# SciML/NonlinearSolve.jl

Hardware: AMD Instinct MI355X
Metric: newton_steps_per_sec (higher is better)
Workload: dtype f64; 1 GPU; bratu2d_1024x1024_newtonraphson_gmres30_fixedwork_csr_spmv; unknowns_global=1048576, unknowns_per_gpu=1048576, arnoldi_steps_per_newton_step=30, ortho=sstep_auto_auto, parallelism=row-range x1, comm=none

## Files before the change

nonlinearsolve.jl_amd/csrc/nk_powers.hip:

```cpp
#include <algorithm>
#include <stdlib.h>
#include <vector>

#include "nk_internal.h"

constexpr int PW_T = 1024;
constexpr int PW_HALO = 1024;
constexpr int PW_FLAG_STRIDE = 16;
constexpr int PW_NXCD = 8;

struct pw_args {
  int nrows, nb, s, stall;
  const int32_t *rowptr, *col;
  const double *val;
  const double *x0;
  double *Y;
  int64_t ldy;
  const double *scal_first, *scal_rest, *theta;
  const int *d_skip;
  uint64_t *flags;
  uint64_t base;
  uint64_t *err;
  int ns;
  double c_lap;
  const double *diag;
  int seg_len, ring;
  struct {
    int up, dn;
    const int32_t *halo_vl;
    double *push_up, *push_dn;
    uint64_t *flag_up, *flag_dn;
    const double *recv_up, *recv_dn;
    const uint64_t *myflag_up, *myflag_dn;
    uint64_t *err;
    int ebuf;
  } pr;
};

constexpr int PW_NST = 12, PW_STP = 16;
__device__ unsigned long long *g_pw_stamp = nullptr;
#ifdef NK_PW_STAMPS
#define PW_STAMP(p, i) do { if (t == 0 && (p) < PW_STP) s_pw_st[(p) * PW_NST + (i)] = wall_clock64(); } while (0)
#else
#define PW_STAMP(p, i) do { } while (0)
#endif

__device__ __forceinline__ int pw_band_of(int bid, int nb) {
  const int q = nb / PW_NXCD, r = nb % PW_NXCD;
  const int x = bid % PW_NXCD, k = bid / PW_NXCD;
  return x * q + (x < r ? x : r) + k;
}
__device__ __forceinline__ void pw_store_sc1(double *p, double v) {
  __hip_atomic_store(reinterpret_cast<unsigned long long *>(p), (unsigned long long)__double_as_longlong(v), __ATOMIC_RELAXED,
                     __HIP_MEMORY_SCOPE_AGENT);
}
__device__ __forceinline__ double pw_load_sc1(const double *p) {
  return __longlong_as_double((long long)__hip_atomic_load(reinterpret_cast<const unsigned long long *>(p), __ATOMIC_RELAXED,
                                                           __HIP_MEMORY_SCOPE_AGENT));
}
__device__ __forceinline__ bool pw_wait(const uint64_t *f, uint64_t target, uint64_t *err) {
  if (__hip_atomic_load(f, __ATOMIC_RELAXED, __HIP_MEMORY_SCOPE_AGENT) >= target) return true;
  const unsigned long long t0 = wall_clock64(), lim = err[1];
  for (unsigned it = 1;; ++it) {
    __builtin_amdgcn_s_sleep(1);
    if (__hip_atomic_load(f, __ATOMIC_RELAXED, __HIP_MEMORY_SCOPE_AGENT) >= target) return true;
    if ((it & 63u) == 0) {
      if (__hip_atomic_load(err, __ATOMIC_RELAXED, __HIP_MEMORY_SCOPE_SYSTEM) != 0) return false;
      if (wall_clock64() - t0 > lim) {
        __hip_atomic_store(err, (uint64_t)1, __ATOMIC_RELAXED, __HIP_MEMORY_SCOPE_SYSTEM);
        return false;
      }
    }
  }
}
__device__ __forceinline__ bool pw_wait_peer(const uint64_t *f, uint64_t target, uint64_t *perr, uint64_t *err) {
  if (__hip_atomic_load(f, __ATOMIC_ACQUIRE, __HIP_MEMORY_SCOPE_SYSTEM) >= target) return true;
  const unsigned long long t0 = wall_clock64(), lim = nk_peer_timeout(perr);
  for (unsigned it = 1;; ++it) {
    __builtin_amdgcn_s_sleep(1);
    if (__hip_atomic_load(f, __ATOMIC_ACQUIRE, __HIP_MEMORY_SCOPE_SYSTEM) >= target) return true;
    if ((it & 63u) == 0) {
      if (__hip_atomic_load(err, __ATOMIC_RELAXED, __HIP_MEMORY_SCOPE_SYSTEM) != 0) return false;
      if (__hip_atomic_load(perr, __ATOMIC_RELAXED, __HIP_MEMORY_SCOPE_AGENT) > 4 || wall_clock64() - t0 > lim) {
        atomicAdd((unsigned long long *)perr, 1ull);
        __hip_atomic_store(err, (uint64_t)1, __ATOMIC_RELAXED, __HIP_MEMORY_SCOPE_SYSTEM);
        return false;
      }
    }
  }
}
__device__ __forceinline__ void pw_store_sys(double *p, double v) {
  __hip_atomic_store(reinterpret_cast<unsigned long long *>(p), (unsigned long long)__double_as_longlong(v), __ATOMIC_RELAXED,
                     __HIP_MEMORY_SCOPE_SYSTEM);
}
__device__ __forceinline__ double pw_load_sys(const double *p) {
  return __longlong_as_double((long long)__hip_atomic_load(reinterpret_cast<const unsigned long long *>(p), __ATOMIC_RELAXED,
                                                           __HIP_MEMORY_SCOPE_SYSTEM));
}
__device__ __forceinline__ double pw_uniform(double x) {
  const unsigned long long u = (unsigned long long)__double_as_longlong(x);
  const unsigned lo = __builtin_amdgcn_readfirstlane((unsigned)u), hi = __builtin_amdgcn_readfirstlane((unsigned)(u >> 32));
  return __longlong_as_double((long long)(((unsigned long long)hi << 32) | lo));
}
template <int RPT>
__device__ __forceinline__ constexpr int pw_slice(int q) {
  return q == 0 ? 0 : (q == 1 ? RPT - 1 : q - 1);
}

template <int RPT, int W, int GEN, bool PEER = false>
__global__ __launch_bounds__(PW_T) void k_spmv_powers(const pw_args a) {
  if (a.d_skip != nullptr && *a.d_skip != 0) return;
  extern __shared__ double pw_x[];
  __shared__ int s_abort;
#ifdef NK_PW_STAMPS
  __shared__ unsigned long long s_pw_st[PW_STP * PW_NST];
  for (int i = threadIdx.x; i < PW_STP * PW_NST; i += PW_T) s_pw_st[i] = 0;
#endif
  constexpr int RB = PW_T * RPT, XN = RB + 2 * PW_HALO;
  constexpr int NBND = RPT > 1 ? 2 : 1;
  const int t = threadIdx.x;
  const int b = pw_band_of(blockIdx.x, a.nb);
  const int r0 = b * RB;
  double *xa = pw_x, *xb = pw_x + XN;
  const bool pup = PEER && b == 0 && a.pr.up != 0, pdn = PEER && b == a.nb - 1 && a.pr.dn != 0;

  double v[RPT][W];
  int ci[RPT][W];
  int len[RPT];
  if constexpr (GEN == 1) {
    static_assert(W >= 5, "the 5-point stencil needs five slots per row");
#pragma unroll
    for (int i = 0; i < RPT; ++i) {
      const int r = r0 + t + PW_T * i;
      const int rc = r < a.nrows ? r : a.nrows - 1;
      const int gj = rc / a.ns, gi = rc - gj * a.ns;
      const double dd = a.diag[rc];
      const int base = rc - (r0 - PW_HALO), own = PW_HALO + t + PW_T * i;
      const bool hs = gj > 0, hw = gi > 0, he = gi + 1 < a.ns, hn = gj + 1 < a.ns;
      const int pW = hs ? 1 : 0, pC = pW + (hw ? 1 : 0), pE = pC + 1, pN = pE + (he ? 1 : 0), n = pN + (hn ? 1 : 0);
      const double off = -a.c_lap, ctr = 4.0 * a.c_lap - dd;
#pragma unroll
      for (int j = 0; j < W; ++j) {
        double vv = 0.0;
        int cc = own;
        if (hs && j == 0) { vv = off; cc = base - a.ns; }
        if (hw && j == pW) { vv = off; cc = base - 1; }
        if (j == pC) { vv = ctr; cc = base; }
        if (he && j == pE) { vv = off; cc = base + 1; }
        if (hn && j == pN) { vv = off; cc = base + a.ns; }
        v[i][j] = vv;
        ci[i][j] = cc;
      }
      len[i] = r < a.nrows ? n : 0;
    }
  } else if constexpr (W > 8) {
#pragma unroll
    for (int i = 0; i < RPT; ++i) {
      const int r = r0 + t + PW_T * i;
      const int rc = r < a.nrows ? r : a.nrows - 1;
      const int k0 = a.rowptr[rc], k1 = a.rowptr[rc + 1];
      len[i] = r < a.nrows ? k1 - k0 : 0;
#pragma unroll
      for (int j = 0; j < W; ++j) {
        v[i][j] = a.val[k0 + j];
        int c = a.col[k0 + j];
        if (PEER && (pup || pdn) && j < len[i] && c >= a.nrows) c = a.pr.halo_vl[c - a.nrows];
        ci[i][j] = (j < len[i]) ? c - (r0 - PW_HALO) : PW_HALO + t + PW_T * i;
      }
    }
  } else {
    double *sv = pw_x;
    int *sc = reinterpret_cast<int *>(pw_x + (size_t)PW_T * W);
#pragma unroll
    for (int i = 0; i < RPT; ++i) {
      const int rfirst = r0 + PW_T * i;
      const int r = rfirst + t;
      const int rc = r < a.nrows ? r : a.nrows - 1;
      const int k0 = a.rowptr[rc], k1 = a.rowptr[rc + 1];
      const int rl = rfirst < a.nrows ? (rfirst + PW_T <= a.nrows ? rfirst + PW_T : a.nrows) : rfirst;
      const int kb = rfirst < a.nrows ? a.rowptr[rfirst] : 0, ke = rfirst < a.nrows ? a.rowptr[rl] : 0;
      len[i] = r < a.nrows ? k1 - k0 : 0;
#pragma unroll
      for (int j = 0; j < W; ++j) {
        const int e = t + PW_T * j;
        if (kb + e < ke) { sv[e] = a.val[kb + e]; sc[e] = a.col[kb + e]; }
      }
      __syncthreads();
#pragma unroll
      for (int j = 0; j < W; ++j) {
        const int e = (j < len[i]) ? k0 - kb + j : 0;
        const double vv = sv[e];
        int c = sc[e];
        if (PEER && (pup || pdn) && j < len[i] && c >= a.nrows) c = a.pr.halo_vl[c - a.nrows];
        v[i][j] = (j < len[i]) ? vv : 0.0;
        ci[i][j] = (j < len[i]) ? c - (r0 - PW_HALO) : PW_HALO + t + PW_T * i;
      }
      __syncthreads();
    }
  }
  for (int idx = t; idx < XN; idx += PW_T) {
    const int g = r0 - PW_HALO + idx;
    xa[idx] = (g >= 0 && g < a.nrows) ? a.x0[g] : 0.0;
    xb[idx] = 0.0;
  }
  if (t == 0) s_abort = 0;
  __syncthreads();
  if (PEER && (pup || pdn)) {
    if (pup) pw_store_sys(a.pr.push_up + (size_t)a.pr.ebuf * PW_T + t, a.x0[t]);
    if (pdn) pw_store_sys(a.pr.push_dn + (size_t)a.pr.ebuf * PW_T + t, a.x0[a.nrows - PW_T + t]);
    __threadfence_system();
    __syncthreads();
    if (t == 0 && pup) __hip_atomic_store(a.pr.flag_up, a.base, __ATOMIC_RELEASE, __HIP_MEMORY_SCOPE_SYSTEM);
    if (t == 64 && pdn) __hip_atomic_store(a.pr.flag_dn, a.base, __ATOMIC_RELEASE, __HIP_MEMORY_SCOPE_SYSTEM);
    if (t == 0 && pup && !pw_wait_peer(a.pr.myflag_up, a.base, a.pr.err, a.err)) s_abort = 1;
    if (t == 64 && pdn && !pw_wait_peer(a.pr.myflag_dn, a.base, a.pr.err, a.err)) s_abort = 1;
    __syncthreads();
    if (s_abort) return;
    if (pup) xa[t] = pw_load_sys(a.pr.recv_up + (size_t)a.pr.ebuf * PW_T + t);
    if (pdn) xa[PW_HALO + RB + t] = pw_load_sys(a.pr.recv_dn + (size_t)a.pr.ebuf * PW_T + t);
    __syncthreads();
  }

  const bool shifted = a.theta != nullptr;
  const double os_first = pw_uniform(a.scal_first ? *a.scal_first : 1.0), os_rest = pw_uniform(a.scal_rest ? *a.scal_rest : 1.0);
  double th = pw_uniform(shifted ? a.theta[0] : 0.0);
  for (int p = 0; p < a.s; ++p) {
    const double *xin = (p & 1) ? xb : xa;
    double *xout = (p & 1) ? xa : xb;
    const double *osp = (p == 0) ? a.scal_first : a.scal_rest;
    const double os = (p == 0) ? os_first : os_rest;
    double *ycol = a.Y + (int64_t)p * a.ldy;
    const bool pub = p + 1 < a.s;
    const size_t boff = (size_t)(a.pr.ebuf + ((p + 1) & 1)) * PW_T + t;
    PW_STAMP(p, 0);
#pragma unroll
    for (int q = 0; q < RPT; ++q) {
      const int i = pw_slice<RPT>(q);
      const int lr = t + PW_T * i, r = r0 + lr;
      constexpr bool BATCH = RPT * W < 30;
      double xv[BATCH ? W : 1], xo = 0.0;
      if constexpr (BATCH) {
#pragma unroll
        for (int j = 0; j < W; ++j) xv[j] = xin[ci[i][j]];
        xo = xin[PW_HALO + lr];
        __builtin_amdgcn_sched_barrier(0);
      }
      double sum = 0.0;
#pragma unroll
      for (int j = 0; j < W; ++j) {
        double xj;
        if constexpr (BATCH) xj = xv[j]; else xj = xin[ci[i][j]];
        const double pr = v[i][j] * xj;
        sum = (j < len[i]) ? sum + pr : sum;
      }
      if constexpr (!BATCH) xo = xin[PW_HALO + lr];
      double out = shifted ? sum - th * xo : sum;
      out = osp ? os * out : out;
      if (r < a.nrows) {
        xout[PW_HALO + lr] = out;
        if (q < NBND) pw_store_sc1(ycol + r, out);
        else ycol[r] = out;
      }
      if (PEER && pub) {
        if (pup && i == 0) pw_store_sys(a.pr.push_up + boff, out);
        if (pdn && i == RPT - 1) pw_store_sys(a.pr.push_dn + boff, out);
      }
      if (q == NBND - 1) PW_STAMP(p, 1);
      if (pub && q == NBND - 1) {
        if (PEER && (pup || pdn)) __threadfence_system();
        asm volatile("s_waitcnt vmcnt(0)" ::: "memory");
        PW_STAMP(p, 2);
        __syncthreads();
        PW_STAMP(p, 3);
        if (t == 0 && !(a.stall && b == 0))
          __hip_atomic_store(a.flags + (size_t)b * PW_FLAG_STRIDE, a.base + (uint64_t)p + 1, __ATOMIC_RELAXED,
                             __HIP_MEMORY_SCOPE_AGENT);
        if (PEER) {
          if (t == 64 && pup) __hip_atomic_store(a.pr.flag_up, a.base + (uint64_t)p + 1, __ATOMIC_RELEASE, __HIP_MEMORY_SCOPE_SYSTEM);
          if (t == 128 && pdn) __hip_atomic_store(a.pr.flag_dn, a.base + (uint64_t)p + 1, __ATOMIC_RELEASE, __HIP_MEMORY_SCOPE_SYSTEM);
        }
      }
    }
    PW_STAMP(p, 4);
    if (!pub) break;
    if (t == 0) {
      if (b > 0) {
        if (!pw_wait(a.flags + (size_t)(b - 1) * PW_FLAG_STRIDE, a.base + (uint64_t)p + 1, a.err)) s_abort = 1;
      } else if (PEER && pup) {
        if (!pw_wait_peer(a.pr.myflag_up, a.base + (uint64_t)p + 1, a.pr.err, a.err)) s_abort = 1;
      }
    }
    PW_STAMP(p, 5);
    if (t == 64) {
      if (b + 1 < a.nb) {
        if (!pw_wait(a.flags + (size_t)(b + 1) * PW_FLAG_STRIDE, a.base + (uint64_t)p + 1, a.err)) s_abort = 1;
      } else if (PEER && pdn) {
        if (!pw_wait_peer(a.pr.myflag_dn, a.base + (uint64_t)p + 1, a.pr.err, a.err)) s_abort = 1;
      }
    }
    __syncthreads();
    PW_STAMP(p, 6);
    if (s_abort) return;
    {
      const int gu = r0 - PW_HALO + t, gd = r0 + RB + t;
      double hu = 0.0, hd = 0.0;
      if (b > 0) hu = pw_load_sc1(ycol + gu);
      else if (PEER && pup) hu = pw_load_sys(a.pr.recv_up + boff);
      if (gd < a.nrows) hd = pw_load_sc1(ycol + gd);
      else if (PEER && pdn) hd = pw_load_sys(a.pr.recv_dn + boff);
      th = pw_uniform(shifted ? a.theta[p + 1] : 0.0);
#ifdef NK_PW_STAMPS
      asm volatile("s_waitcnt vmcnt(0)" ::: "memory");
      PW_STAMP(p, 7);
#endif
      xout[t] = hu;
      xout[PW_HALO + RB + t] = hd;
    }
    __syncthreads();
    PW_STAMP(p, 9);
  }
#ifdef NK_PW_STAMPS
  __syncthreads();
  if (g_pw_stamp != nullptr)
    for (int i = t; i < PW_STP * PW_NST; i += PW_T) g_pw_stamp[(size_t)b * PW_STP * PW_NST + i] = s_pw_st[i];
#endif
}

template <int RPS, int W, int SEG>
__global__ __launch_bounds__(PW_T) void k_spmv_powers_seg(const pw_args a) {
  if (a.d_skip != nullptr && *a.d_skip != 0) return;
  extern __shared__ double pw_x[];
  __shared__ int s_abort;
  constexpr int RB = PW_T * RPS, XS = RB + 2 * PW_HALO, XN = SEG * XS, NSL = SEG * RPS;
  static_assert(W <= 8, "the slices are staged through LDS");
  const int t = threadIdx.x;
  const int b = pw_band_of(blockIdx.x, a.nb);
  const int M = a.seg_len, b0 = b * RB;
  const bool ring = a.ring != 0;
  double *xa = pw_x, *xb = pw_x + XN;

  double v[NSL][W];
  int ci[NSL][W];
  int len[NSL];
  {
    double *sv = pw_x;
    int *sc = reinterpret_cast<int *>(pw_x + (size_t)PW_T * W);
#pragma unroll
    for (int i = 0; i < NSL; ++i) {
      const int sg = i / RPS, j = i % RPS;
      const int lfirst = b0 + PW_T * j;
      const bool any = lfirst < M;
      const bool valid = lfirst + t < M;
      const int rfirst = sg * M + lfirst, r = rfirst + t;
      const int rc = valid ? r : (any ? sg * M + M - 1 : 0);
      const int k0 = a.rowptr[rc], k1 = a.rowptr[rc + 1];
      const int rl = any ? sg * M + (lfirst + PW_T <= M ? lfirst + PW_T : M) : 0;
      const int kb = any ? a.rowptr[rfirst] : 0, ke = any ? a.rowptr[rl] : 0;
      len[i] = valid ? k1 - k0 : 0;
#pragma unroll
      for (int jj = 0; jj < W; ++jj) {
        const int e = t + PW_T * jj;
        if (kb + e < ke) { sv[e] = a.val[kb + e]; sc[e] = a.col[kb + e]; }
      }
      __syncthreads();
#pragma unroll
      for (int jj = 0; jj < W; ++jj) {
        const int e = (jj < len[i]) ? k0 - kb + jj : 0;
        const double vv = sv[e];
        const int c = sc[e];
        const int sgc = SEG > 1 ? c / M : 0;
        int d = c - sgc * M - b0;
        if (ring) d = d < -PW_HALO ? d + M : (d >= RB + PW_HALO ? d - M : d);
        v[i][jj] = (jj < len[i]) ? vv : 0.0;
        ci[i][jj] = (jj < len[i]) ? sgc * XS + PW_HALO + d : sg * XS + PW_HALO + PW_T * j + t;
      }
      __syncthreads();
    }
  }
  for (int idx = t; idx < XN; idx += PW_T) {
    const int sg = idx / XS;
    int l = b0 - PW_HALO + (idx - sg * XS);
    if (ring) l = l < 0 ? l + M : (l >= M ? l - M : l);
    xa[idx] = (l >= 0 && l < M) ? a.x0[sg * M + l] : 0.0;
    xb[idx] = 0.0;
  }
  if (t == 0) s_abort = 0;
  __syncthreads();

  const bool shifted = a.theta != nullptr;
  const int nup = b > 0 ? b - 1 : (ring ? a.nb - 1 : -1), ndn = b + 1 < a.nb ? b + 1 : (ring ? 0 : -1);
  for (int p = 0; p < a.s; ++p) {
    const double *xin = (p & 1) ? xb : xa;
    double *xout = (p & 1) ? xa : xb;
    const double *osp = (p == 0) ? a.scal_first : a.scal_rest;
    const double os = osp ? *osp : 1.0;
    const double th = shifted ? a.theta[p] : 0.0;
    double *ycol = a.Y + (int64_t)p * a.ldy;
    const bool pub = p + 1 < a.s;
#pragma unroll
    for (int i = 0; i < NSL; ++i) {
      const int sg = i / RPS, j = i % RPS;
      const int lrow = b0 + PW_T * j + t, own = sg * XS + PW_HALO + PW_T * j + t;
      double sum = 0.0;
#pragma unroll
      for (int jj = 0; jj < W; ++jj) {
        const double pr = v[i][jj] * xin[ci[i][jj]];
        sum = (jj < len[i]) ? sum + pr : sum;
      }
      double out = shifted ? sum - th * xin[own] : sum;
      out = osp ? os * out : out;
      if (lrow < M) {
        xout[own] = out;
        if (pub && (j == 0 || j == RPS - 1)) pw_store_sc1(ycol + sg * M + lrow, out);
        else ycol[sg * M + lrow] = out;
      }
    }
    if (!pub) break;
    asm volatile("s_waitcnt vmcnt(0)" ::: "memory");
    __syncthreads();
    if (t == 0 && !(a.stall && b == 0))
      __hip_atomic_store(a.flags + (size_t)b * PW_FLAG_STRIDE, a.base + (uint64_t)p + 1, __ATOMIC_RELAXED, __HIP_MEMORY_SCOPE_AGENT);
    if (t == 0 && nup >= 0) {
      if (!pw_wait(a.flags + (size_t)nup * PW_FLAG_STRIDE, a.base + (uint64_t)p + 1, a.err)) s_abort = 1;
    }
    if (t == 64 && ndn >= 0) {
      if (!pw_wait(a.flags + (size_t)ndn * PW_FLAG_STRIDE, a.base + (uint64_t)p + 1, a.err)) s_abort = 1;
    }
    __syncthreads();
    if (s_abort) return;
    {
      double hu[SEG], hd[SEG];
      int lu = b0 - PW_HALO + t, ld = b0 + RB + t;
      if (ring) { lu = lu < 0 ? lu + M : lu; ld = ld >= M ? ld - M : ld; }
#pragma unroll
      for (int sg = 0; sg < SEG; ++sg) {
        hu[sg] = (nup >= 0 && lu >= 0 && lu < M) ? pw_load_sc1(ycol + sg * M + lu) : 0.0;
        hd[sg] = (ndn >= 0 && ld < M) ? pw_load_sc1(ycol + sg * M + ld) : 0.0;
      }
#pragma unroll
      for (int sg = 0; sg < SEG; ++sg) {
        xout[sg * XS + t] = hu[sg];
        xout[sg * XS + PW_HALO + RB + t] = hd[sg];
      }
    }
    __syncthreads();
  }
}

struct nk_powers_plan {
  int rpt = 0, w = 0, nb = 0;
  int seg = 0, ring = 0, seg_len = 0;
  uint64_t *d_flags = nullptr;
  uint64_t *h_err = nullptr, *h_err_dev = nullptr;
  uint64_t epoch = 0;
  bool broken = false;
  int strikes = 0;
  bool peer = false;
  nk_peer_powers pp;
  int32_t *d_halo_vl = nullptr;
};
void nk_powers_plan_destroy(nk_powers_plan *P) {
  if (!P) return;
  hipFree(P->d_flags);
  hipFree(P->d_halo_vl);
  if (P->h_err) hipHostFree(P->h_err);
  delete P;
}
static int pw_stall_hook() {
  static const std::vector<long> stalls = [] {
    std::vector<long> v;
    const char *e = getenv("NK_PW_DEBUG_STALL_LAUNCH");
    while (e && *e) {
      char *end = nullptr;
      const long x = strtol(e, &end, 10);
      if (end == e) break;
      v.push_back(x);
      e = (*end == ',') ? end + 1 : end;
    }
    return v;
  }();
  static long launches = 0;
  ++launches;
  bool stall = false;
  for (long x : stalls) stall = stall || (x > 0 && launches == x);
  return stall ? 1 : 0;
}
static bool pw_enabled() {
  static const bool on = !(getenv("NK_SPMV_POWERS") && atoi(getenv("NK_SPMV_POWERS")) == 0);
  return on;
}

template <int RPT, int W, int GEN, bool PEER = false>
static int pw_launch(nk_ctx *ctx, const pw_args &a, bool query, int *occ) {
  constexpr size_t lds_x = (size_t)2 * (PW_T * RPT + 2 * PW_HALO) * sizeof(double), lds_m = (W > 8 || GEN == 1) ? 0 : (size_t)PW_T * W * 12;
  constexpr size_t lds = lds_x > lds_m ? lds_x : lds_m;
  if (lds > 64 * 1024)
    NK_HIP(hipFuncSetAttribute(reinterpret_cast<const void *>(&k_spmv_powers<RPT, W, GEN, PEER>),
                               hipFuncAttributeMaxDynamicSharedMemorySize, (int)lds));
  if (query) {
    NK_HIP(hipOccupancyMaxActiveBlocksPerMultiprocessor(occ, k_spmv_powers<RPT, W, GEN, PEER>, PW_T, lds));
    return NK_OK;
  }
  hipEvent_t e0 = nullptr, e1 = nullptr;
  if (ctx->prof.on && nk_prof_next(ctx, &e0, &e1))
    hipExtLaunchKernelGGL((k_spmv_powers<RPT, W, GEN, PEER>), dim3(a.nb), dim3(PW_T), lds, ctx->stream, e0, e1, 0, a);
  else
    hipLaunchKernelGGL((k_spmv_powers<RPT, W, GEN, PEER>), dim3(a.nb), dim3(PW_T), lds, ctx->stream, a);
  NK_HIP(hipGetLastError());
  return NK_OK;
}
static int pw_dispatch(nk_ctx *ctx, int rpt, int w, const pw_args &a, bool query, int *occ, int gen = 0, bool peer = false) {
  if (peer) {
#define PW_PEER(R, WW) if (rpt == R && w == WW) return pw_launch<R, WW, 0, true>(ctx, a, query, occ)
    PW_PEER(1, 5); PW_PEER(2, 5); PW_PEER(4, 5); PW_PEER(6, 5);
    PW_PEER(1, 8); PW_PEER(2, 8);
    PW_PEER(1, 16);
#undef PW_PEER
    NK_FAIL(NK_E_INVALID, "internal: no matrix-powers kernel for %d rows per thread × %d entries per row", rpt, w);
  }
#define PW_CASE(R, WW, G) if (rpt == R && w == WW && gen == G) return pw_launch<R, WW, G>(ctx, a, query, occ)
  PW_CASE(1, 5, 1); PW_CASE(2, 5, 1); PW_CASE(4, 5, 1); PW_CASE(6, 5, 1);
  PW_CASE(1, 5, 0); PW_CASE(2, 5, 0); PW_CASE(4, 5, 0); PW_CASE(6, 5, 0);
  PW_CASE(1, 8, 0); PW_CASE(2, 8, 0);
  PW_CASE(1, 16, 0);
#undef PW_CASE
  NK_FAIL(NK_E_INVALID, "internal: no matrix-powers kernel for %d rows per thread × %d entries per row", rpt, w);
}

template <int RPS, int W, int SEG>
static int pw_launch_seg(nk_ctx *ctx, const pw_args &a, bool query, int *occ) {
  constexpr size_t lds_x = (size_t)2 * SEG * (PW_T * RPS + 2 * PW_HALO) * sizeof(double), lds_m = (size_t)PW_T * W * 12;
  constexpr size_t lds = lds_x > lds_m ? lds_x : lds_m;
  if (lds > 64 * 1024)
    NK_HIP(hipFuncSetAttribute(reinterpret_cast<const void *>(&k_spmv_powers_seg<RPS, W, SEG>), hipFuncAttributeMaxDynamicSharedMemorySize,
                               (int)lds));
  if (query) {
    NK_HIP(hipOccupancyMaxActiveBlocksPerMultiprocessor(occ, k_spmv_powers_seg<RPS, W, SEG>, PW_T, lds));
    return NK_OK;
  }
  hipEvent_t e0 = nullptr, e1 = nullptr;
  if (ctx->prof.on && nk_prof_next(ctx, &e0, &e1))
    hipExtLaunchKernelGGL((k_spmv_powers_seg<RPS, W, SEG>), dim3(a.nb), dim3(PW_T), lds, ctx->stream, e0, e1, 0, a);
  else
    hipLaunchKernelGGL((k_spmv_powers_seg<RPS, W, SEG>), dim3(a.nb), dim3(PW_T), lds, ctx->stream, a);
  NK_HIP(hipGetLastError());
  return NK_OK;
}
static bool pw_seg_shape(int rps, int w, int seg) {
  if (seg == 1) return (w == 5 && (rps == 1 || rps == 2 || rps == 4)) || (w == 8 && (rps == 1 || rps == 2));
  if (seg == 2) return (w == 5 && (rps == 1 || rps == 2)) || (w == 8 && rps == 1);
  return false;
}
static int pw_dispatch_seg(nk_ctx *ctx, int rps, int w, int seg, const pw_args &a, bool query, int *occ) {
#define PW_SEG(R, WW, SG) if (rps == R && w == WW && seg == SG) return pw_launch_seg<R, WW, SG>(ctx, a, query, occ)
  PW_SEG(1, 5, 1); PW_SEG(2, 5, 1); PW_SEG(4, 5, 1); PW_SEG(1, 8, 1); PW_SEG(2, 8, 1);
  PW_SEG(1, 5, 2); PW_SEG(2, 5, 2); PW_SEG(1, 8, 2);
#undef PW_SEG
  NK_FAIL(NK_E_INVALID, "internal: no segmented matrix-powers kernel for %d slices × %d slots × %d segments", rps, w, seg);
}

static int pw_plan_new(nk_ctx *ctx, int rpt, int w, int nb, nk_powers_plan **out) {
  nk_powers_plan *P = new nk_powers_plan();
  auto guard = nk_make_guard(P, [](nk_powers_plan *p) { nk_powers_plan_destroy(p); });
  P->rpt = rpt; P->w = w; P->nb = nb;
  NK_TRY(nk_dev_alloc(&P->d_flags, (size_t)nb * PW_FLAG_STRIDE));
  NK_HIP(nk_memset(ctx, P->d_flags, 0, (size_t)nb * PW_FLAG_STRIDE * sizeof(uint64_t)));
  NK_HIP(hipHostMalloc((void **)&P->h_err, 2 * sizeof(uint64_t), hipHostMallocMapped | hipHostMallocCoherent));
  NK_HIP(hipHostGetDevicePointer((void **)&P->h_err_dev, P->h_err, 0));
  P->h_err[0] = 0;
  {
    const char *e = getenv("NK_PW_TIMEOUT_MS");
    const double ms = e ? atof(e) : 250.0;
    P->h_err[1] = (uint64_t)((ms > 1.0 ? ms : 1.0) * 1.0e5);
  }
  *out = guard.release();
  return NK_OK;
}

struct pw_layout {
  int kind = 0;
  int rpt = 0, w = 0, nb = 0, seg = 0, ring = 0;
  int64_t M = 0;
};
static pw_layout pw_find_layout(int64_t n, const int32_t *rowptr, const int32_t *col, int num_cus, int skip) {
  pw_layout L;
  if (n < 1 || num_cus < 1) return L;
  int maxlen = 0;
  for (int64_t r = 0; r < n; ++r) maxlen = std::max(maxlen, (int)(rowptr[r + 1] - rowptr[r]));
  const int w = maxlen <= 5 ? 5 : (maxlen <= 8 ? 8 : (maxlen <= 16 ? 16 : 0));
  if (!w) return L;
  for (int lay = skip; lay < 4; ++lay) {
    if (lay == 0) {
      const int64_t per_cu = (n + num_cus - 1) / num_cus;
      const int need = (int)((per_cu + PW_T - 1) / PW_T);
      const int rpt = need <= 1 ? 1 : (need <= 2 ? 2 : (need <= 4 ? 4 : (need <= 6 ? 6 : 0)));
      if (!rpt) continue;
      if ((w == 8 && rpt > 2) || (w == 16 && rpt > 1)) continue;
      const int64_t rb = (int64_t)PW_T * rpt;
      bool ok = true;
      for (int64_t r = 0; r < n && ok; ++r) {
        const int64_t b0 = (r / rb) * rb, lo = b0 - PW_HALO, hi = b0 + rb + PW_HALO;
        for (int32_t k = rowptr[r]; k < rowptr[r + 1]; ++k)
          if (col[k] < lo || col[k] >= hi) { ok = false; break; }
      }
      if (!ok) continue;
      L.kind = 1; L.rpt = rpt; L.w = w; L.nb = (int)((n + rb - 1) / rb); L.seg = 1; L.ring = 0; L.M = n;
      return L;
    }
    const int seg = lay == 1 ? 1 : 2, ring = lay == 2 ? 0 : 1;
    if (n % seg) continue;
    const int64_t M = n / seg, pc = (M + num_cus - 1) / num_cus;
    const int nd = (int)((pc + PW_T - 1) / PW_T);
    const int rps = nd <= 1 ? 1 : (nd <= 2 ? 2 : (nd <= 4 ? 4 : 0));
    if (!rps || !pw_seg_shape(rps, w, seg)) continue;
    const int64_t RB = (int64_t)PW_T * rps;
    if (ring && (M % RB)) continue;
    bool ok = true;
    for (int64_t r = 0; r < n && ok; ++r) {
      const int64_t b0 = ((r % M) / RB) * RB;
      for (int32_t k = rowptr[r]; k < rowptr[r + 1]; ++k) {
        if (col[k] < 0 || col[k] >= n) { ok = false; break; }
        int64_t d = (int64_t)col[k] % M - b0;
        if (ring) d = d < -PW_HALO ? d + M : (d >= RB + PW_HALO ? d - M : d);
        if (d < -PW_HALO || d >= RB + PW_HALO) { ok = false; break; }
      }
    }
    if (!ok) continue;
    L.kind = 2; L.rpt = rps; L.w = w; L.nb = (int)((M + RB - 1) / RB); L.seg = seg; L.ring = ring; L.M = M;
    return L;
  }
  return L;
}
static int pw_layout_index(const pw_layout &L) { return L.kind == 1 ? 0 : (L.seg == 1 ? 1 : (L.ring ? 3 : 2)); }
extern "C" int nk_csr_powers_layout(int64_t nrows, const int32_t *rowptr, const int32_t *col, int num_cus, int layout[6]) {
  NK_REQUIRE(rowptr && col && layout && nrows >= 0 && num_cus >= 1, "bad argument");
  const pw_layout L = pw_find_layout(nrows, rowptr, col, num_cus, 0);
  layout[0] = L.kind; layout[1] = L.rpt; layout[2] = L.w; layout[3] = L.nb; layout[4] = L.seg; layout[5] = L.ring;
  return NK_OK;
}

static int pw_plan_ranks(nk_csr *A) {
  nk_ctx *ctx = A->ctx;
  const int64_t n = A->nrows;
  const int nh = (int)A->halo_gcols.size();
  std::vector<int32_t> hvl(nh > 0 ? nh : 1, 0), vcol;
  bool ok = pw_enabled() && ctx->peer.on && !ctx->device_shared && n >= PW_T && A->nnz >= 1;
  static const bool ranks_off = getenv("NK_PW_RANKS") && atoi(getenv("NK_PW_RANKS")) == 0;
  ok = ok && !ranks_off;
  for (int h = 0; h < nh && ok; ++h) {
    const int64_t vl = A->halo_gcols[h] - A->row_begin;
    ok = (vl < 0 && vl >= -PW_HALO && ctx->rank > 0) || (vl >= n && vl < n + PW_HALO && ctx->rank + 1 < ctx->nranks);
    hvl[h] = (int32_t)vl;
  }
  pw_layout L;
  if (ok) {
    vcol.resize(A->h_col.size());
    for (size_t k = 0; k < vcol.size(); ++k) vcol[k] = A->h_col[k] < n ? A->h_col[k] : hvl[A->h_col[k] - n];
    L = pw_find_layout(n, A->h_rowptr.data(), vcol.data(), ctx->num_cus, 0);
    ok = L.kind == 1 && n % ((int64_t)PW_T * L.rpt) == 0;
    if (ok) {
      pw_args probe{};
      int occ = 0;
      NK_TRY(pw_dispatch(ctx, L.rpt, L.w, probe, true, &occ, 0, true));
      ok = occ >= 1 && L.nb <= ctx->num_cus * occ;
    }
  }
  nk_peer_powers pp;
  bool all = false;
  NK_TRY(nk_peer_powers_setup(ctx, ok, &pp, &all));
  if (!all) return NK_OK;
  NK_TRY(pw_plan_new(A->ctx, L.rpt, L.w, L.nb, &A->pw));
  A->pw->peer = true;
  A->pw->pp = pp;
  NK_HIP(hipMalloc((void **)&A->pw->d_halo_vl, hvl.size() * sizeof(int32_t)));
  NK_HIP(nk_memcpy(ctx, A->pw->d_halo_vl, hvl.data(), hvl.size() * sizeof(int32_t), hipMemcpyHostToDevice));
  return NK_OK;
}
static int pw_plan(nk_csr *A) {
  if (A->pw_tried) return NK_OK;
  A->pw_tried = true;
  nk_ctx *ctx = A->ctx;
  if (ctx->nranks > 1 && A->local_only) return NK_OK;
  if (ctx->nranks > 1) return pw_plan_ranks(A);
  if (!pw_enabled() || !A->halo_gcols.empty() || A->nrows < 1 || A->nnz < 1) return NK_OK;
  pw_args probe{};
  for (int skip = 0; skip < 4;) {
    const pw_layout L = pw_find_layout(A->nrows, A->h_rowptr.data(), A->h_col.data(), ctx->num_cus, skip);
    if (!L.kind) return NK_OK;
    int occ = 0;
    if (L.kind == 1) NK_TRY(pw_dispatch(ctx, L.rpt, L.w, probe, true, &occ));
    else NK_TRY(pw_dispatch_seg(ctx, L.rpt, L.w, L.seg, probe, true, &occ));
    if (occ >= 1 && L.nb <= ctx->num_cus * occ) {
      NK_TRY(pw_plan_new(A->ctx, L.rpt, L.w, L.nb, &A->pw));
      if (L.kind == 2) { A->pw->seg = L.seg; A->pw->ring = L.ring; A->pw->seg_len = (int)L.M; }
      return NK_OK;
    }
    skip = pw_layout_index(L) + 1;
  }
  return NK_OK;
}
bool nk_csr_powers_ready(nk_csr *A) {
  if (!A->pw_tried && pw_plan(A) != NK_OK) return false;
  return A->pw != nullptr && !A->pw->broken && A->pw->h_err[0] == 0;
}
int nk_csr_powers_check(nk_csr *A) {
  if (!A->pw || A->pw->broken || A->pw->h_err[0] == 0) return NK_OK;
  A->pw->broken = true;
  A->pw->strikes++;
  NK_FAIL(NK_E_HIP, "resident matrix-powers kernel: a workgroup waited longer than NK_PW_TIMEOUT_MS for its neighbour band "
                    "(NK_SPMV_POWERS=0 keeps the streaming SpMV)");
}
static void pw_rearm(nk_powers_plan *P) {
  if (!P || !P->broken || P->peer || P->strikes >= 3) return;
  P->h_err[0] = 0;
  P->broken = false;
}
void nk_csr_powers_rearm(nk_csr *A) { if (A) pw_rearm(A->pw); }
void nk_problem_powers_rearm(nk_problem *P) { if (P) pw_rearm(P->pw); }
int nk_csr_powers_dev(nk_csr *A, const double *d_x0, double *d_Y, int64_t ldy, int s, const double *d_scal_first,
                      const double *d_scal_rest, const double *d_theta, const int *d_skip) {
  NK_REQUIRE(nk_csr_powers_ready(A), "internal: matrix powers on a matrix without a plan");
  NK_REQUIRE(s >= 1 && s <= 200, "matrix powers: 1 ≤ s ≤ 200");
  nk_ctx *ctx = A->ctx;
  nk_powers_plan *P = A->pw;
  pw_args a{};
  a.nrows = (int)A->nrows; a.nb = P->nb; a.s = s; a.stall = pw_stall_hook();
  a.rowptr = A->d_rowptr; a.col = A->d_col; a.val = A->d_val;
  a.x0 = d_x0; a.Y = d_Y; a.ldy = ldy;
  a.scal_first = d_scal_first; a.scal_rest = d_scal_rest; a.theta = d_theta; a.d_skip = d_skip;
  a.flags = P->d_flags; a.base = (++P->epoch) << 8; a.err = P->h_err_dev;
  ctx->stats.op_applies += s;
  nk_prof_scope prof_(ctx, NK_K_POWERS,
                      (double)s * (12.0 * (double)A->nnz + 4.0 * (double)(A->nrows + 1) + 16.0 * (double)A->nrows));
  if (P->seg > 0) {
    a.seg_len = P->seg_len; a.ring = P->ring;
    return pw_dispatch_seg(ctx, P->rpt, P->w, P->seg, a, false, nullptr);
  }
  if (P->peer) {
    a.pr.up = ctx->rank > 0; a.pr.dn = ctx->rank + 1 < ctx->nranks;
    a.pr.halo_vl = P->d_halo_vl;
    a.pr.push_up = P->pp.push_up; a.pr.push_dn = P->pp.push_dn; a.pr.flag_up = P->pp.flag_up; a.pr.flag_dn = P->pp.flag_dn;
    a.pr.recv_up = P->pp.recv_up; a.pr.recv_dn = P->pp.recv_dn; a.pr.myflag_up = P->pp.myflag_up; a.pr.myflag_dn = P->pp.myflag_dn;
    a.pr.err = nk_peer_err_ptr(ctx);
    a.pr.ebuf = (int)(P->epoch & 1) * 2;
    ctx->stats.halo_exchanges++;
    return pw_dispatch(ctx, P->rpt, P->w, a, false, nullptr, 0, true);
  }
  return pw_dispatch(ctx, P->rpt, P->w, a, false, nullptr);
}

static int pw_problem_plan(nk_problem *P) {
  if (P->pw_tried) return NK_OK;
  P->pw_tried = true;
  nk_ctx *ctx = P->ctx;
  if (!pw_enabled() || P->kind != NK_PROBLEM_BRATU2D || ctx->nranks != 1 || P->replicated || P->j0 != 0 || P->j1 != P->ns ||
      P->ns < 2 || P->ns > PW_HALO || P->n_local != P->ns * P->ns)
    return NK_OK;
  const int64_t n = P->n_local, per_cu = (n + ctx->num_cus - 1) / ctx->num_cus;
  const int need = (int)((per_cu + PW_T - 1) / PW_T);
  const int rpt = need <= 1 ? 1 : (need <= 2 ? 2 : (need <= 4 ? 4 : (need <= 6 ? 6 : 0)));
  if (!rpt) return NK_OK;
  const int nb = (int)((n + (int64_t)PW_T * rpt - 1) / ((int64_t)PW_T * rpt));
  pw_args probe{};
  int occ = 0;
  NK_TRY(pw_dispatch(ctx, rpt, 5, probe, true, &occ, 1));
  if (occ < 1 || nb > ctx->num_cus * occ) return NK_OK;
  return pw_plan_new(P->ctx, rpt, 5, nb, &P->pw);
}
bool nk_problem_powers_ready(nk_problem *P) {
  if (!P->pw_tried && pw_problem_plan(P) != NK_OK) return false;
  return P->pw != nullptr && !P->pw->broken && P->pw->h_err[0] == 0;
}
int nk_problem_powers_check(nk_problem *P) {
  if (!P->pw || P->pw->broken || P->pw->h_err[0] == 0) return NK_OK;
  P->pw->broken = true;
  P->pw->strikes++;
  NK_FAIL(NK_E_HIP, "resident matrix-powers kernel (matrix-free): a workgroup waited longer than NK_PW_TIMEOUT_MS for its "
                    "neighbour band (NK_SPMV_POWERS=0 keeps the per-column JVP)");
}
int nk_problem_powers_dev(nk_problem *P, const double *d_u, const double *d_x0, double *d_Y, int64_t ldy, int s,
                          const double *d_scal_first, const double *d_scal_rest, const double *d_theta, const int *d_skip) {
  NK_REQUIRE(nk_problem_powers_ready(P), "internal: matrix powers on a problem without a plan");
  nk_ctx *ctx = P->ctx;
  if (P->d_u_lin != d_u || !P->d_diag) NK_TRY(nk_problem_jvp_prepare(P, d_u));
  nk_powers_plan *Q = P->pw;
  pw_args a{};
  a.nrows = (int)P->n_local; a.nb = Q->nb; a.s = s; a.stall = pw_stall_hook();
  a.x0 = d_x0; a.Y = d_Y; a.ldy = ldy;
  a.scal_first = d_scal_first; a.scal_rest = d_scal_rest; a.theta = d_theta; a.d_skip = d_skip;
  a.flags = Q->d_flags; a.base = (++Q->epoch) << 8; a.err = Q->h_err_dev;
  a.ns = (int)P->ns; a.c_lap = P->c_lap; a.diag = P->d_diag;
  ctx->stats.op_applies += s;
  nk_prof_scope prof_(ctx, NK_K_POWERS, (double)s * 24.0 * (double)P->n_local);
  return pw_dispatch(ctx, Q->rpt, 5, a, false, nullptr, 1);
}

extern "C" int nk_csr_powers(nk_csr *A, const double *x, double *Y, int64_t ldy, int s, const double *theta, double scale,
                             int memspace, int *resident) {
  NK_REQUIRE(A && x && Y && s >= 1 && s <= 64 && ldy >= A->nrows, "bad argument");
  nk_ctx *ctx = A->ctx;
  NK_HIP(hipSetDevice(ctx->device));
  const int64_t n = A->nrows;
  double *dx = nullptr, *dY = nullptr, *dsc = nullptr;
  auto cleanup = [&]() { if (memspace != NK_DEVICE) { hipFree(dx); hipFree(dY); } hipFree(dsc); };
  if (memspace == NK_DEVICE) { dx = const_cast<double *>(x); dY = Y; }
  else {
    NK_TRY(nk_dev_alloc(&dx, (size_t)n));
    if (nk_dev_alloc(&dY, (size_t)ldy * s) != NK_OK) { cleanup(); return NK_E_NOMEM; }
    NK_HIP(nk_memcpy(ctx, dx, x, n * sizeof(double), hipMemcpyHostToDevice));
  }
  if (nk_dev_alloc(&dsc, (size_t)s + 1) != NK_OK) { cleanup(); return NK_E_NOMEM; }
  std::vector<double> hs((size_t)s + 1, 0.0);
  hs[0] = scale;
  if (theta) for (int p = 0; p < s; ++p) hs[1 + p] = theta[p];
  nk_memcpy(ctx, dsc, hs.data(), hs.size() * sizeof(double), hipMemcpyHostToDevice);
  nk_csr_powers_rearm(A);
  const bool res = nk_csr_powers_ready(A);
  bool res_used = res;
  int rc = NK_OK;
  auto streaming = [&]() -> int {
    int r = NK_OK;
    for (int p = 0; p < s && r == NK_OK; ++p) {
      nk_spmv_epi ep;
      if (theta) { ep.mode = NK_EPI_SHIFTED; ep.theta = dsc + 1 + p; }
      r = nk_csr_spmv_dev(A, p == 0 ? dx : dY + (size_t)(p - 1) * ldy, dY + (size_t)p * ldy, nullptr, dsc, &ep);
    }
    return r;
  };
  rc = res ? nk_csr_powers_dev(A, dx, dY, ldy, s, dsc, dsc, theta ? dsc + 1 : nullptr, nullptr) : streaming();
  if (rc == NK_OK && hipStreamSynchronize(ctx->stream) != hipSuccess) { nk_set_error("stream error in nk_csr_powers"); rc = NK_E_HIP; }
  if (rc == NK_OK && res && nk_csr_powers_check(A) != NK_OK) {
    res_used = false;
    rc = streaming();
    if (rc == NK_OK && hipStreamSynchronize(ctx->stream) != hipSuccess) { nk_set_error("stream error in nk_csr_powers"); rc = NK_E_HIP; }
  }
  if (rc == NK_OK && memspace != NK_DEVICE)
    if (nk_memcpy(ctx, Y, dY, (size_t)ldy * s * sizeof(double), hipMemcpyDeviceToHost) != hipSuccess) rc = NK_E_HIP;
  cleanup();
  if (resident) *resident = res_used ? 1 : 0;
  return rc;
}

extern "C" int nk_pw_debug_stamps(int enable, unsigned long long *out, int nbands) {
  static unsigned long long *d_st = nullptr;
  const size_t words = (size_t)1024 * PW_STP * PW_NST;
  if (enable && !d_st) {
    if (hipMalloc(&d_st, words * sizeof(unsigned long long)) != hipSuccess) return NK_E_NOMEM;
    hipMemset(d_st, 0, words * sizeof(unsigned long long));
    hipDeviceSynchronize();
    hipMemcpyToSymbol(HIP_SYMBOL(g_pw_stamp), &d_st, sizeof(d_st));
  }
  if (!enable && d_st) {
    unsigned long long *z = nullptr;
    hipMemcpyToSymbol(HIP_SYMBOL(g_pw_stamp), &z, sizeof(z));
  }
  if (out && d_st && nbands > 0 && nbands <= 1024) {
    hipDeviceSynchronize();
    hipMemcpy(out, d_st, (size_t)nbands * PW_STP * PW_NST * sizeof(unsigned long long), hipMemcpyDeviceToHost);
  }
  return NK_OK;
}
```

Before: 2460 newton_steps/s.

## Precompute packed 16-bit LDS column offsets for matrix-powers kernel setup

After: 2541 newton_steps/s (median of 6 runs). +3.3%, better.

```diff
diff --git a/nonlinearsolve.jl_amd/csrc/nk_powers.hip b/nonlinearsolve.jl_amd/csrc/nk_powers.hip
--- a/nonlinearsolve.jl_amd/csrc/nk_powers.hip
+++ b/nonlinearsolve.jl_amd/csrc/nk_powers.hip
@@ -3,15 +3,16 @@
 #include <vector>
 
 #include "nk_internal.h"
-
-constexpr int PW_T = 1024;
-constexpr int PW_HALO = 1024;
+#include "nk_pw_pack.h"
+
 constexpr int PW_FLAG_STRIDE = 16;
 constexpr int PW_NXCD = 8;
 
 struct pw_args {
   int nrows, nb, s, stall;
   const int32_t *rowptr, *col;
+  const uint32_t *rec;
+  const int32_t *ext;
   const double *val;
   const double *x0;
   double *Y;
@@ -27,7 +28,6 @@
   int seg_len, ring;
   struct {
     int up, dn;
-    const int32_t *halo_vl;
     double *push_up, *push_dn;
     uint64_t *flag_up, *flag_dn;
     const double *recv_up, *recv_dn;
@@ -123,6 +123,7 @@
   const int r0 = b * RB;
   double *xa = pw_x, *xb = pw_x + XN;
   const bool pup = PEER && b == 0 && a.pr.up != 0, pdn = PEER && b == a.nb - 1 && a.pr.dn != 0;
+  PW_STAMP(0, 10);
 
   double v[RPT][W];
   int ci[RPT][W];
@@ -153,55 +154,76 @@
       }
       len[i] = r < a.nrows ? n : 0;
     }
-  } else if constexpr (W > 8) {
+  } else {
+    using F = pw_rec<W>;
+    constexpr int NW = F::NW;
+    static_assert(F::OFF_MAX >= (uint32_t)XN - 1, "an LDS offset of the band's window fits its field");
+    const uint32_t *rp = a.rec + (size_t)b * RPT * NW * PW_T + t;
+    const int32_t *ex = a.ext + (size_t)b * RPT * 2;
+    uint32_t rec[RPT][NW];
+#pragma unroll
+    for (int i = 0; i < RPT; ++i)
+#pragma unroll
+      for (int k = 0; k < NW; ++k) rec[i][k] = rp[(size_t)(i * NW + k) * PW_T];
+    double x0r[RPT + 2];
+#pragma unroll
+    for (int k = 0; k < RPT + 2; ++k) {
+      const int g = r0 - PW_HALO + t + PW_T * k;
+      x0r[k] = (g >= 0 && g < a.nrows) ? a.x0[g] : 0.0;
+    }
+    if constexpr (W > 8) {
+#pragma unroll
+      for (int i = 0; i < RPT; ++i) {
+        const int k0 = ex[2 * i] + F::start(rec[i]), n = F::len(rec[i]);
+#pragma unroll
+        for (int j = 0; j < W; ++j) v[i][j] = (j < n) ? a.val[k0 + j] : 0.0;
+      }
+    } else {
+      constexpr int NBUF = RPT > 1 ? 2 : 1;
+      double tv[W];
+      auto request = [&](int i) {
+        const int kb = ex[2 * i], ke = ex[2 * i + 1];
+#pragma unroll
+        for (int j = 0; j < W; ++j) {
+          const int e = t + PW_T * j;
+          tv[j] = (kb + e < ke) ? a.val[kb + e] : 0.0;
+        }
+      };
+      request(0);
+#pragma unroll
+      for (int i = 0; i < RPT; ++i) {
+        double *sv = pw_x + (size_t)(i % NBUF) * PW_T * W;
+#pragma unroll
+        for (int j = 0; j < W; ++j) sv[t + PW_T * j] = tv[j];
+        if (i + 1 < RPT) request(i + 1);
+        __syncthreads();
+        const int k0 = F::start(rec[i]), n = F::len(rec[i]);
+#pragma unroll
+        for (int j = 0; j < W; ++j) {
+          const double vv = sv[(j < n) ? k0 + j : 0];
+          v[i][j] = (j < n) ? vv : 0.0;
+        }
+      }
+    }
 #pragma unroll
     for (int i = 0; i < RPT; ++i) {
-      const int r = r0 + t + PW_T * i;
-      const int rc = r < a.nrows ? r : a.nrows - 1;
-      const int k0 = a.rowptr[rc], k1 = a.rowptr[rc + 1];
-      len[i] = r < a.nrows ? k1 - k0 : 0;
-#pragma unroll
-      for (int j = 0; j < W; ++j) {
-        v[i][j] = a.val[k0 + j];
-        int c = a.col[k0 + j];
-        if (PEER && (pup || pdn) && j < len[i] && c >= a.nrows) c = a.pr.halo_vl[c - a.nrows];
-        ci[i][j] = (j < len[i]) ? c - (r0 - PW_HALO) : PW_HALO + t + PW_T * i;
-      }
-    }
-  } else {
-    double *sv = pw_x;
-    int *sc = reinterpret_cast<int *>(pw_x + (size_t)PW_T * W);
-#pragma unroll
-    for (int i = 0; i < RPT; ++i) {
-      const int rfirst = r0 + PW_T * i;
-      const int r = rfirst + t;
-      const int rc = r < a.nrows ? r : a.nrows - 1;
-      const int k0 = a.rowptr[rc], k1 = a.rowptr[rc + 1];
-      const int rl = rfirst < a.nrows ? (rfirst + PW_T <= a.nrows ? rfirst + PW_T : a.nrows) : rfirst;
-      const int kb = rfirst < a.nrows ? a.rowptr[rfirst] : 0, ke = rfirst < a.nrows ? a.rowptr[rl] : 0;
-      len[i] = r < a.nrows ? k1 - k0 : 0;
-#pragma unroll
-      for (int j = 0; j < W; ++j) {
-        const int e = t + PW_T * j;
-        if (kb + e < ke) { sv[e] = a.val[kb + e]; sc[e] = a.col[kb + e]; }
-      }
-      __syncthreads();
-#pragma unroll
-      for (int j = 0; j < W; ++j) {
-        const int e = (j < len[i]) ? k0 - kb + j : 0;
-        const double vv = sv[e];
-        int c = sc[e];
-        if (PEER && (pup || pdn) && j < len[i] && c >= a.nrows) c = a.pr.halo_vl[c - a.nrows];
-        v[i][j] = (j < len[i]) ? vv : 0.0;
-        ci[i][j] = (j < len[i]) ? c - (r0 - PW_HALO) : PW_HALO + t + PW_T * i;
-      }
-      __syncthreads();
-    }
-  }
-  for (int idx = t; idx < XN; idx += PW_T) {
-    const int g = r0 - PW_HALO + idx;
-    xa[idx] = (g >= 0 && g < a.nrows) ? a.x0[g] : 0.0;
-    xb[idx] = 0.0;
+      len[i] = F::len(rec[i]);
+#pragma unroll
+      for (int j = 0; j < W; ++j) ci[i][j] = F::off(rec[i], j);
+    }
+    __syncthreads();
+#pragma unroll
+    for (int k = 0; k < RPT + 2; ++k) {
+      xa[t + PW_T * k] = x0r[k];
+      xb[t + PW_T * k] = 0.0;
+    }
+  }
+  if constexpr (GEN == 1) {
+    for (int idx = t; idx < XN; idx += PW_T) {
+      const int g = r0 - PW_HALO + idx;
+      xa[idx] = (g >= 0 && g < a.nrows) ? a.x0[g] : 0.0;
+      xb[idx] = 0.0;
+    }
   }
   if (t == 0) s_abort = 0;
   __syncthreads();
@@ -457,12 +479,14 @@
   int strikes = 0;
   bool peer = false;
   nk_peer_powers pp;
-  int32_t *d_halo_vl = nullptr;
+  uint32_t *d_rec = nullptr;
+  int32_t *d_ext = nullptr;
 };
 void nk_powers_plan_destroy(nk_powers_plan *P) {
   if (!P) return;
   hipFree(P->d_flags);
-  hipFree(P->d_halo_vl);
+  hipFree(P->d_rec);
+  hipFree(P->d_ext);
   if (P->h_err) hipHostFree(P->h_err);
   delete P;
 }
@@ -492,8 +516,10 @@
 
 template <int RPT, int W, int GEN, bool PEER = false>
 static int pw_launch(nk_ctx *ctx, const pw_args &a, bool query, int *occ) {
-  constexpr size_t lds_x = (size_t)2 * (PW_T * RPT + 2 * PW_HALO) * sizeof(double), lds_m = (W > 8 || GEN == 1) ? 0 : (size_t)PW_T * W * 12;
+  constexpr size_t lds_x = (size_t)2 * (PW_T * RPT + 2 * PW_HALO) * sizeof(double);
+  constexpr size_t lds_m = (W > 8 || GEN == 1) ? 0 : (size_t)(RPT > 1 ? 2 : 1) * PW_T * W * sizeof(double);
   constexpr size_t lds = lds_x > lds_m ? lds_x : lds_m;
+  static_assert(lds <= 160 * 1024, "the CU's LDS");
   if (lds > 64 * 1024)
     NK_HIP(hipFuncSetAttribute(reinterpret_cast<const void *>(&k_spmv_powers<RPT, W, GEN, PEER>),
                                hipFuncAttributeMaxDynamicSharedMemorySize, (int)lds));
@@ -574,6 +600,13 @@
     P->h_err[1] = (uint64_t)((ms > 1.0 ? ms : 1.0) * 1.0e5);
   }
   *out = guard.release();
+  return NK_OK;
+}
+static int pw_plan_table(nk_ctx *ctx, nk_powers_plan *P, const pw_pack_out &T) {
+  NK_HIP(hipMalloc((void **)&P->d_rec, T.rec.size() * sizeof(uint32_t)));
+  NK_HIP(hipMalloc((void **)&P->d_ext, T.ext.size() * sizeof(int32_t)));
+  NK_HIP(nk_memcpy(ctx, P->d_rec, T.rec.data(), T.rec.size() * sizeof(uint32_t), hipMemcpyHostToDevice));
+  NK_HIP(nk_memcpy(ctx, P->d_ext, T.ext.data(), T.ext.size() * sizeof(int32_t), hipMemcpyHostToDevice));
   return NK_OK;
 }
 
@@ -632,6 +665,12 @@
   return L;
 }
 static int pw_layout_index(const pw_layout &L) { return L.kind == 1 ? 0 : (L.seg == 1 ? 1 : (L.ring ? 3 : 2)); }
+static bool pw_pack_plain(const nk_csr *A, const pw_layout &L, const int32_t *hvl, int nh, pw_pack_out *T) {
+  pw_pack_in in;
+  in.n = A->nrows; in.rowptr = A->h_rowptr.data(); in.col = A->h_col.data();
+  in.rpt = L.rpt; in.w = L.w; in.nb = L.nb; in.hvl = hvl; in.nh = nh;
+  return pw_pack(in, T) == PW_PACK_OK;
+}
 extern "C" int nk_csr_powers_layout(int64_t nrows, const int32_t *rowptr, const int32_t *col, int num_cus, int layout[6]) {
   NK_REQUIRE(rowptr && col && layout && nrows >= 0 && num_cus >= 1, "bad argument");
   const pw_layout L = pw_find_layout(nrows, rowptr, col, num_cus, 0);
@@ -665,6 +704,8 @@
       ok = occ >= 1 && L.nb <= ctx->num_cus * occ;
     }
   }
+  pw_pack_out table;
+  ok = ok && pw_pack_plain(A, L, hvl.data(), nh, &table);
   nk_peer_powers pp;
   bool all = false;
   NK_TRY(nk_peer_powers_setup(ctx, ok, &pp, &all));
@@ -672,9 +713,7 @@
   NK_TRY(pw_plan_new(A->ctx, L.rpt, L.w, L.nb, &A->pw));
   A->pw->peer = true;
   A->pw->pp = pp;
-  NK_HIP(hipMalloc((void **)&A->pw->d_halo_vl, hvl.size() * sizeof(int32_t)));
-  NK_HIP(nk_memcpy(ctx, A->pw->d_halo_vl, hvl.data(), hvl.size() * sizeof(int32_t), hipMemcpyHostToDevice));
-  return NK_OK;
+  return pw_plan_table(ctx, A->pw, table);
 }
 static int pw_plan(nk_csr *A) {
   if (A->pw_tried) return NK_OK;
@@ -691,8 +730,11 @@
     if (L.kind == 1) NK_TRY(pw_dispatch(ctx, L.rpt, L.w, probe, true, &occ));
     else NK_TRY(pw_dispatch_seg(ctx, L.rpt, L.w, L.seg, probe, true, &occ));
     if (occ >= 1 && L.nb <= ctx->num_cus * occ) {
+      pw_pack_out table;
+      if (L.kind == 1 && !pw_pack_plain(A, L, nullptr, 0, &table)) return NK_OK;
       NK_TRY(pw_plan_new(A->ctx, L.rpt, L.w, L.nb, &A->pw));
       if (L.kind == 2) { A->pw->seg = L.seg; A->pw->ring = L.ring; A->pw->seg_len = (int)L.M; }
+      else NK_TRY(pw_plan_table(ctx, A->pw, table));
       return NK_OK;
     }
     skip = pw_layout_index(L) + 1;
@@ -700,7 +742,11 @@
   return NK_OK;
 }
 bool nk_csr_powers_ready(nk_csr *A) {
-  if (!A->pw_tried && pw_plan(A) != NK_OK) return false;
+  if (!A->pw_tried && pw_plan(A) != NK_OK) {
+    nk_powers_plan_destroy(A->pw);
+    A->pw = nullptr;
+    return false;
+  }
   return A->pw != nullptr && !A->pw->broken && A->pw->h_err[0] == 0;
 }
 int nk_csr_powers_check(nk_csr *A) {
@@ -726,6 +772,7 @@
   pw_args a{};
   a.nrows = (int)A->nrows; a.nb = P->nb; a.s = s; a.stall = pw_stall_hook();
   a.rowptr = A->d_rowptr; a.col = A->d_col; a.val = A->d_val;
+  a.rec = P->d_rec; a.ext = P->d_ext;
   a.x0 = d_x0; a.Y = d_Y; a.ldy = ldy;
   a.scal_first = d_scal_first; a.scal_rest = d_scal_rest; a.theta = d_theta; a.d_skip = d_skip;
   a.flags = P->d_flags; a.base = (++P->epoch) << 8; a.err = P->h_err_dev;
@@ -738,7 +785,6 @@
   }
   if (P->peer) {
     a.pr.up = ctx->rank > 0; a.pr.dn = ctx->rank + 1 < ctx->nranks;
-    a.pr.halo_vl = P->d_halo_vl;
     a.pr.push_up = P->pp.push_up; a.pr.push_dn = P->pp.push_dn; a.pr.flag_up = P->pp.flag_up; a.pr.flag_dn = P->pp.flag_dn;
     a.pr.recv_up = P->pp.recv_up; a.pr.recv_dn = P->pp.recv_dn; a.pr.myflag_up = P->pp.myflag_up; a.pr.myflag_dn = P->pp.myflag_dn;
     a.pr.err = nk_peer_err_ptr(ctx);
diff --git a/nonlinearsolve.jl_amd/csrc/nk_pw_pack.h b/nonlinearsolve.jl_amd/csrc/nk_pw_pack.h
--- /dev/null
+++ b/nonlinearsolve.jl_amd/csrc/nk_pw_pack.h
@@ -0,0 +1,99 @@
+#pragma once
+#include <cstddef>
+#include <cstdint>
+#include <vector>
+
+#if defined(__HIPCC__)
+#define PW_HD __host__ __device__
+#else
+#define PW_HD
+#endif
+
+constexpr int PW_T = 1024;
+constexpr int PW_HALO = 1024;
+constexpr int PW_START_BITS_ODD = 13;
+
+template <int W>
+struct pw_rec {
+  static constexpr bool LEN_IN_H0 = (W % 2) == 1;
+  static constexpr int NH = W + 1 + (LEN_IN_H0 ? 0 : 1);
+  static constexpr int NW = NH / 2;
+  static constexpr uint32_t START_MAX = LEN_IN_H0 ? (1u << PW_START_BITS_ODD) - 1 : 0xFFFFu;
+  static constexpr uint32_t LEN_MAX = LEN_IN_H0 ? (1u << (16 - PW_START_BITS_ODD)) - 1 : 0xFFFFu;
+  static constexpr uint32_t OFF_MAX = 0xFFFFu;
+  static_assert(NH % 2 == 0, "whole words");
+  static_assert(START_MAX >= (uint32_t)PW_T * W, "the row-start field holds every position of a staged slice");
+  static_assert(LEN_MAX >= (uint32_t)W, "the length field holds W");
+  PW_HD static uint32_t half(const uint32_t *w, int h) { return (w[h >> 1] >> ((h & 1) * 16)) & 0xFFFFu; }
+  PW_HD static int start(const uint32_t *w) { return (int)(half(w, 0) & START_MAX); }
+  PW_HD static int len(const uint32_t *w) { return LEN_IN_H0 ? (int)(half(w, 0) >> PW_START_BITS_ODD) : (int)half(w, W + 1); }
+  PW_HD static int off(const uint32_t *w, int j) { return (int)half(w, 1 + j); }
+};
+inline int pw_rec_words(int w) { return (w + 1 + ((w % 2) ? 0 : 1)) / 2; }
+
+struct pw_pack_in {
+  int64_t n = 0;
+  const int32_t *rowptr = nullptr;
+  const int32_t *col = nullptr;
+  int rpt = 0, w = 0, nb = 0;
+  const int32_t *hvl = nullptr;
+  int nh = 0;
+};
+struct pw_pack_out {
+  std::vector<uint32_t> rec;
+  std::vector<int32_t> ext;
+};
+enum { PW_PACK_OK = 0, PW_PACK_E_ARG = 1, PW_PACK_E_LEN = 2, PW_PACK_E_RANGE = 3, PW_PACK_E_HALO = 4, PW_PACK_E_EXTENT = 5 };
+
+inline int pw_pack(const pw_pack_in &in, pw_pack_out *out) {
+  const int w = in.w, rpt = in.rpt;
+  if (!out || !in.rowptr || !in.col || in.n < 1 || rpt < 1 || (w != 5 && w != 8 && w != 16) || in.nh < 0) return PW_PACK_E_ARG;
+  const int64_t rb = (int64_t)PW_T * rpt, xn = rb + 2 * PW_HALO;
+  if (xn - 1 > 0xFFFF || in.nb < 1 || (int64_t)in.nb != (in.n + rb - 1) / rb) return PW_PACK_E_ARG;
+  const bool len_in_h0 = (w % 2) == 1;
+  const uint32_t start_max = len_in_h0 ? (1u << PW_START_BITS_ODD) - 1 : 0xFFFFu;
+  const int nw = pw_rec_words(w);
+  out->rec.assign((size_t)in.nb * rpt * nw * PW_T, 0u);
+  out->ext.assign((size_t)in.nb * rpt * 2, 0);
+  for (int b = 0; b < in.nb; ++b)
+    for (int i = 0; i < rpt; ++i) {
+      const int64_t r0 = (int64_t)b * rb, rfirst = r0 + (int64_t)PW_T * i;
+      const bool any = rfirst < in.n;
+      const int64_t rl = any ? (rfirst + PW_T <= in.n ? rfirst + PW_T : in.n) : rfirst;
+      const int32_t kb = any ? in.rowptr[rfirst] : 0, ke = any ? in.rowptr[rl] : 0;
+      if (kb < 0 || ke < kb || (int64_t)ke - kb > (int64_t)PW_T * w) return PW_PACK_E_EXTENT;
+      out->ext[((size_t)b * rpt + i) * 2] = kb;
+      out->ext[((size_t)b * rpt + i) * 2 + 1] = ke;
+      uint32_t *slice = out->rec.data() + ((size_t)b * rpt + i) * nw * PW_T;
+      for (int t = 0; t < PW_T; ++t) {
+        const int64_t r = rfirst + t;
+        const uint32_t own = (uint32_t)(PW_HALO + t + PW_T * i);
+        uint32_t h[18] = {};
+        int len = 0;
+        uint32_t start = 0;
+        if (r < in.n) {
+          const int32_t k0 = in.rowptr[r], k1 = in.rowptr[r + 1];
+          if (k1 < k0 || k1 - k0 > w) return PW_PACK_E_LEN;
+          if (k0 < kb || k1 > ke || (uint32_t)(k0 - kb) > start_max) return PW_PACK_E_EXTENT;
+          len = k1 - k0;
+          start = (uint32_t)(k0 - kb);
+          for (int j = 0; j < len; ++j) {
+            int64_t c = in.col[k0 + j];
+            if (c < 0) return PW_PACK_E_RANGE;
+            if (c >= in.n) {
+              if (!in.hvl || c - in.n >= in.nh) return PW_PACK_E_HALO;
+              c = in.hvl[c - in.n];
+            }
+            const int64_t o = c - (r0 - PW_HALO);
+            if (o < 0 || o >= xn) return PW_PACK_E_RANGE;
+            h[1 + j] = (uint32_t)o;
+          }
+        }
+        for (int j = len; j < w; ++j) h[1 + j] = own;
+        if (len_in_h0) h[0] = start | ((uint32_t)len << PW_START_BITS_ODD);
+        else { h[0] = start; h[w + 1] = (uint32_t)len; }
+        for (int k = 0; k < nw; ++k) slice[(size_t)k * PW_T + t] = h[2 * k] | (h[2 * k + 1] << 16);
+      }
+    }
+  return PW_PACK_OK;
+}
```
